# loop-Z/omniisaacgymenvs_loop

Hardware: AMD Instinct MI355X
Metric: env-steps/sec USV_CaptureXY at 1/2/4/8 MI355X; wall-clock to reward=30 (higher is better)
Workload: dtype fp32; 1 GPU; USV_Virtual_CaptureXY num_envs=131072/GPU PPO-MLP fp32 (BASELINE configs[4] per GPU: 2^20 envs over 8 GPUs); num_envs_per_gpu=131072, horizon_length=16, minibatch_size=8192, mini_epochs=8, parallelism=dp1, exchange=none (one rank), seed=0, full=False

## Files before the change

### omniisaacgymenvs_loop_amd/csrc/usv_field.hip

```cpp
#include "usv_device.h"

USV_PROBE_DEFINE(field)

namespace {

constexpr int G = USV_GRID;
constexpr int G2 = USV_GRID2;
constexpr int FS = USV_FIELD_STRIDE;
constexpr int T = 10;
constexpr int NT = G / T;
constexpr int kWaveThreads = 256;
constexpr int kMaxIters = 4096;
constexpr int kSlotStride = USV_FIELD_SLOT_STATS;
constexpr int kSlotObst = 160;
static_assert(kSlotObst + 2 * USV_NOBST <= kSlotStride, "slot_stats layout");
constexpr int kFieldPackMinEnvs = 32768;
#ifndef USV_SWEEP_WAVES
#define USV_SWEEP_WAVES 2
#endif
constexpr int kPackGrid = 256 * USV_SWEEP_WAVES;

enum {
  SS_GMIN_F = 0, SS_GMAX_F, SS_ANY_INF,
  SS_JMIN_F_NI, SS_JMAX_F_NI, SS_JMAX_F_ALL,
  SS_JRMIN_I_NI, SS_JRMAX_I_NI, SS_JRMAX_I_ALL,
  SS_INSIDE, SS_ITERS, SS_EXACT
};

__device__ __forceinline__ float wall(const uint32_t *freem, int bit) {
  const uint32_t f = (freem[bit >> 5] >> (bit & 31)) & 1u;
  return __uint_as_float((f - 1u) & 0x7f800000u);
}

constexpr int NTP = NT + 2;
constexpr uint32_t kInfBits = 0x7f800000u;
constexpr uint32_t kOcc = 0xFFFFFFFFu;
enum { E_TOP = 0, E_BOT, E_LEFT, E_RIGHT };
constexpr int kOccColWords = (G + 31) / 32;
__device__ __forceinline__ bool occ_bit(const uint32_t *occ, int r, int cc) {
  return (occ[cc * kOccColWords + (r >> 5)] >> (r & 31)) & 1u;
}

constexpr int kRefSweeps = (G * 3) / 2;
template <int NT>
__device__ __forceinline__ void cost_sweeps_exact(const uint32_t *occ, int ix, int iy, float *A, float *B) {
  const int tid = threadIdx.x;
  for (int q = tid; q < G2; q += NT) A[q] = (q == iy * G + ix) ? 0.f : INFINITY;
  __syncthreads();
  for (int it = 0; it < kRefSweeps; ++it) {
    for (int q = tid; q < G2; q += NT) {
      const int r = q / G, cc = q % G;
      float m = A[q];
#pragma unroll
      for (int dy = -1; dy <= 1; ++dy)
#pragma unroll
        for (int dx = -1; dx <= 1; ++dx) {
          if (!dx && !dy) continue;
          const int rr = r - dy, c2 = cc - dx;
          if (rr < 0 || rr >= G || c2 < 0 || c2 >= G) continue;
          m = fminf(m, A[rr * G + c2] + ((dx && dy) ? 1.414f : 1.0f));
        }
      const bool o = r == 0 || r == G - 1 || cc == 0 || cc == G - 1 || occ_bit(occ, r, cc);
      B[q] = o ? INFINITY : m;
    }
    __syncthreads();
    float *t = A; A = B; B = t;
  }
}

constexpr int kPlaceTB = 256;
__global__ __launch_bounds__(kPlaceTB) void k_field_place(usv_cfg_t c, usv_bufs_t b) {
  if (b.ctl[USV_CTL_PLACE] == 0) return;
  const int n = b.n;
  const int count = min(b.ctl[USV_CTL_RESET_COUNT], n);
  const uint64_t h_seed = (uint64_t)(uint32_t)b.ctl[USV_CTL_H_SEED_LO] | ((uint64_t)(uint32_t)b.ctl[USV_CTL_H_SEED_HI] << 32);
  const uint64_t h_step = (uint64_t)(uint32_t)b.ctl[USV_CTL_H_STEP_LO] | ((uint64_t)(uint32_t)b.ctl[USV_CTL_H_STEP_HI] << 32);
  const float *h_inj = reinterpret_cast<const float *>(
      (uintptr_t)((uint64_t)(uint32_t)b.ctl[USV_CTL_H_INJ_LO] | ((uint64_t)(uint32_t)b.ctl[USV_CTL_H_INJ_HI] << 32)));
  const int lane = threadIdx.x & 63;
  const int waves = (int)gridDim.x * (kPlaceTB / 64);
  for (int slot = (int)blockIdx.x * (kPlaceTB / 64) + (int)(threadIdx.x >> 6); slot < count; slot += waves) {
    const int e = b.reset_ids[slot];
    const float2 oc = place_obstacles(c, e, b.px[e], b.py[e], b.field_old_tgt[e], b.field_old_tgt[n + e], h_seed,
                                      h_step, h_inj);
    if (lane < USV_NOBST) {
      b.obst[(size_t)(2 * lane) * n + e] = oc.x;
      b.obst[(size_t)(2 * lane + 1) * n + e] = oc.y;
    }
  }
}

#define USV_SWEEP_NOTE(hb, m) (chg = __builtin_amdgcn_bitop3_b32(chg, (uint32_t)(hb), (uint32_t)(m), 0xF6))
template <bool kPlace, int TH = T, int TW = T, int NTHR = kWaveThreads>
__device__ __forceinline__ void field_wave_body(const usv_cfg_t &c, const usv_bufs_t &b) {
  constexpr int NTR = G / TH, NTC = G / TW;
  constexpr int NPR = NTR + 2, NPC = NTC + 2;
  constexpr int WC = NTHR / 128;
  static_assert(G % TH == 0 && G % TW == 0 && NTR <= 16 && NTC <= 8 * WC && NTHR % 128 == 0, "sweep tiling");
  static_assert(USV_FIELD_TH == TH && USV_FIELD_TW % TW == 0, "sweep tiles inside the field tiles");
  __shared__ uint32_t occ[G * kOccColWords];
  __shared__ float edgeh[2][NPR * NPC][TW];
  __shared__ float edgev[2][NPR * NPC][TH];
  __shared__ int lastc[NPR * NPC];
  __shared__ float so[2 * USV_NOBST];
  __shared__ float slin[G];
  const int n = b.n;
  const int count = min(b.ctl[USV_CTL_RESET_COUNT], n);
  const int tid = threadIdx.x;
  const int lane = tid & 63, wid = tid >> 6;
  const bool place = kPlace && b.ctl[USV_CTL_PLACE] != 0;
  uint64_t h_seed = 0, h_step = 0;
  const float *h_inj = nullptr;
  if (kPlace) {
    h_seed = (uint64_t)(uint32_t)b.ctl[USV_CTL_H_SEED_LO] | ((uint64_t)(uint32_t)b.ctl[USV_CTL_H_SEED_HI] << 32);
    h_step = (uint64_t)(uint32_t)b.ctl[USV_CTL_H_STEP_LO] | ((uint64_t)(uint32_t)b.ctl[USV_CTL_H_STEP_HI] << 32);
    h_inj = reinterpret_cast<const float *>(
        (uintptr_t)((uint64_t)(uint32_t)b.ctl[USV_CTL_H_INJ_LO] | ((uint64_t)(uint32_t)b.ctl[USV_CTL_H_INJ_HI] << 32)));
  }
  const int quad = tid >> 6, qk = tid & 63;
  const int qr = quad / WC, qc = quad % WC;
  const int qw = min(8, NTC - 8 * qc), qh = min(8, NTR - 8 * qr);
  const bool tile_ok = qk < qw * qh;
  const int tr = tile_ok ? qr * 8 + qk / qw : 0;
  const int tc = tile_ok ? qc * 8 + qk % qw : 0;
  const int r0 = tr * TH, c0 = tc * TW;
  const int tp = (tr + 1) * NPC + tc + 1;
  const float cell = (float)((double)c.map_size / G);
  const float half_map = (float)((double)c.map_size / 2);
  const float inv_r = (float)(1.0 / (double)c.influence_radius);
  for (int q = tid; q < 2 * NPR * NPC * TW; q += NTHR) {
    const int t = (q / TW) % (NPR * NPC);
    const int rr = t / NPC, cc = t % NPC;
    if (rr == 0 || rr == NPR - 1 || cc == 0 || cc == NPC - 1) (&edgeh[0][0][0])[q] = INFINITY;
  }
  for (int q = tid; q < 2 * NPR * NPC * TH; q += NTHR) {
    const int t = (q / TH) % (NPR * NPC);
    const int rr = t / NPC, cc = t % NPC;
    if (rr == 0 || rr == NPR - 1 || cc == 0 || cc == NPC - 1) (&edgev[0][0][0])[q] = INFINITY;
  }
  for (int q = tid; q < NPR * NPC; q += NTHR) lastc[q] = -1000;
  for (int slot = blockIdx.x; slot < count; slot += gridDim.x) {
    USV_PHASE(field, 0);
    const int e = b.reset_ids[slot];
    if (kPlace && place) {
      if (wid == 0) {
        const float2 oc = place_obstacles(c, e, b.px[e], b.py[e], b.field_old_tgt[e], b.field_old_tgt[n + e],
                                          h_seed, h_step, h_inj);
        if (lane < USV_NOBST) {
          so[2 * lane] = oc.x;
          so[2 * lane + 1] = oc.y;
          b.obst[(size_t)(2 * lane) * n + e] = oc.x;
          b.obst[(size_t)(2 * lane + 1) * n + e] = oc.y;
        }
      }
    } else if (tid < 2 * USV_NOBST) {
      so[tid] = b.obst[(size_t)tid * n + e];
    }
    if (tid < G) slin[tid] = grid_coord(b.grid_lin, c.map_size, tid);
    for (int q = tid; q < G * kOccColWords; q += NTHR) occ[q] = 0u;
    __syncthreads();
#ifdef USV_PHASE_PROBE
    if (tid == 0 && blockIdx.x < 4096) g_probe_field[blockIdx.x][12] = wall_clock64();
#endif
    if (tid < 2 * USV_NOBST) b.slot_stats[(size_t)slot * kSlotStride + kSlotObst + tid] = so[tid];
    {
      const float half_m = (float)((double)c.map_size / 2);
      const float cellf = (float)((double)c.map_size / G);
      const int reach = (int)ceilf(c.obstacle_radius / cellf) + 2;
      const int bw = 2 * reach + 1;
      for (int q = tid; q < USV_NOBST * bw * bw; q += NTHR) {
        const int o = q / (bw * bw), k = q % (bw * bw);
        const float ox = so[2 * o], oy = so[2 * o + 1];
        const float ic = (ox + half_m) / cellf - 0.5f, jc = (oy + half_m) / cellf - 0.5f;
        if (!(fabsf(ic) < 4.0f * G && fabsf(jc) < 4.0f * G)) continue;
        const int cc = (int)floorf(ic) - reach + k % bw, r = (int)floorf(jc) - reach + k / bw;
        if (cc < 0 || cc >= G || r < 0 || r >= G) continue;
        const float dx = slin[cc] - ox, dy = slin[r] - oy;
        if (sqrtf(fmaf(dy, dy, dx * dx)) - c.obstacle_radius <= 0.f)
          atomicOr(&occ[cc * kOccColWords + (r >> 5)], 1u << (r & 31));
      }
    }
    __syncthreads();
    USV_PHASE(field, 1);
#ifdef USV_PHASE_PROBE
    if (tid == 0 && blockIdx.x < 4096) g_probe_field[blockIdx.x][13] = clock64();
#endif
    const float tx = b.field_old_tgt[e], ty = b.field_old_tgt[n + e];
    int ix = (int)((tx + half_map) / cell), iy = (int)((ty + half_map) / cell);
    ix = min(max(ix, 0), G - 1);
    iy = min(max(iy, 0), G - 1);
    const bool tgt_free = !occ_bit(occ, iy, ix) && ix > 0 && ix < G - 1 && iy > 0 && iy < G - 1;
    float h[TH + 2][TW + 2];
    if (tile_ok) {
#pragma unroll
      for (int i = 0; i < TH; ++i)
#pragma unroll
        for (int j = 0; j < TW; ++j) {
          const int r = r0 + i, cc = c0 + j;
          const bool border = r == 0 || r == G - 1 || cc == 0 || cc == G - 1;
          const bool o = border || occ_bit(occ, r, cc);
          float init = INFINITY;
          if (o) {
            init = __uint_as_float(kOcc);
          } else if (tgt_free) {
            if (r == iy && cc == ix) init = 0.f;
          } else {
            const int di = r - iy, dj = cc - ix;
            if (abs(di) <= 1 && abs(dj) <= 1 && (di || dj)) init = (di && dj) ? 1.414f : 1.0f;
          }
          h[i + 1][j + 1] = init;
        }
#pragma unroll
      for (int k = 0; k < TW; ++k) {
        edgeh[E_TOP][tp][k] = h[1][k + 1];
        edgeh[E_BOT][tp][k] = h[TH][k + 1];
      }
#pragma unroll
      for (int k = 0; k < TH; ++k) {
        edgev[E_LEFT - 2][tp][k] = h[k + 1][1];
        edgev[E_RIGHT - 2][tp][k] = h[k + 1][TW];
      }
      lastc[tp] = 0;
    }
    __syncthreads();
    int it = 0;
    for (; it < kMaxIters; ++it) {
      int changed = 0;
      uint32_t chg = 0u;
      bool dirty = false;
      if (tile_ok) {
#pragma unroll
        for (int dr = -1; dr <= 1; ++dr)
#pragma unroll
          for (int dc = -1; dc <= 1; ++dc) dirty |= lastc[tp + dr * NPC + dc] >= it - 1;
      }
      if (dirty) {
#pragma unroll
        for (int k = 0; k < TW; ++k) {
          h[0][k + 1] = edgeh[E_BOT][tp - NPC][k];
          h[TH + 1][k + 1] = edgeh[E_TOP][tp + NPC][k];
        }
#pragma unroll
        for (int k = 0; k < TH; ++k) {
          h[k + 1][0] = edgev[E_RIGHT - 2][tp - 1][k];
          h[k + 1][TW + 1] = edgev[E_LEFT - 2][tp + 1][k];
        }
        h[0][0] = edgeh[E_BOT][tp - NPC - 1][TW - 1];
        h[0][TW + 1] = edgeh[E_BOT][tp - NPC + 1][0];
        h[TH + 1][0] = edgeh[E_TOP][tp + NPC - 1][TW - 1];
        h[TH + 1][TW + 1] = edgeh[E_TOP][tp + NPC + 1][0];
#pragma unroll
        for (int L = 0; L < 2 * TH + TW - 2; ++L)
#pragma unroll
          for (int i = 1; i <= TH; ++i) {
            const int j = L - 2 * (i - 1) + 1;
            if (j < 1 || j > TW) continue;
            const int32_t hb = __float_as_int(h[i][j]);
            int32_t m = min(hb, __float_as_int(fabsf(h[i - 1][j - 1]) + 1.414f));
            m = min(m, __float_as_int(fabsf(h[i - 1][j]) + 1.0f));
            m = min(m, __float_as_int(fabsf(h[i - 1][j + 1]) + 1.414f));
            m = min(m, __float_as_int(fabsf(h[i][j - 1]) + 1.0f));
            if (i == 1 || i == TH || j == 1 || j == TW) USV_SWEEP_NOTE(hb, m);
            h[i][j] = __int_as_float(m);
          }
#pragma unroll
        for (int L = 0; L < 2 * TH + TW - 2; ++L)
#pragma unroll
          for (int i = TH; i >= 1; --i) {
            const int j = TW - (L - 2 * (TH - i));
            if (j < 1 || j > TW) continue;
            const int32_t hb = __float_as_int(h[i][j]);
            int32_t m = min(hb, __float_as_int(fabsf(h[i + 1][j + 1]) + 1.414f));
            m = min(m, __float_as_int(fabsf(h[i + 1][j]) + 1.0f));
            m = min(m, __float_as_int(fabsf(h[i + 1][j - 1]) + 1.414f));
            m = min(m, __float_as_int(fabsf(h[i][j + 1]) + 1.0f));
            USV_SWEEP_NOTE(hb, m);
            h[i][j] = __int_as_float(m);
          }
        __asm__("" : "+v"(chg));
        changed = chg != 0u;
        if (changed) {
#pragma unroll
          for (int k = 0; k < TW; ++k) {
            edgeh[E_TOP][tp][k] = h[1][k + 1];
            edgeh[E_BOT][tp][k] = h[TH][k + 1];
          }
#pragma unroll
          for (int k = 0; k < TH; ++k) {
            edgev[E_LEFT - 2][tp][k] = h[k + 1][1];
            edgev[E_RIGHT - 2][tp][k] = h[k + 1][TW];
          }
          lastc[tp] = it;
        }
      }
      if (!__syncthreads_or(changed)) break;
    }
    USV_PHASE(field, 2);
#ifdef USV_PHASE_PROBE
    if (tid == 0 && blockIdx.x < 4096) g_probe_field[blockIdx.x][14] = clock64();
#endif
    constexpr float kPinnedCost = 224.0f;
    float hmax = 0.f;
    if (tile_ok) {
#pragma unroll
      for (int i = 0; i < TH; ++i)
#pragma unroll
        for (int j = 0; j < TW; ++j) {
          const uint32_t hb = __float_as_uint(h[i + 1][j + 1]);
          if (hb < kInfBits) hmax = fmaxf(hmax, h[i + 1][j + 1]);
        }
    }
    const bool exact = __syncthreads_or((hmax > kPinnedCost) || (it >= kMaxIters)) != 0;
    constexpr int kSub = USV_FIELD_TW / TW;
    static_assert(USV_FIELD_TCOLS * USV_FIELD_TW == G && USV_FIELD_TCOLS == NTC / kSub, "field tiles = sweep tiles");
    if (tile_ok) {
      float *Ft = b.field + (size_t)e * FS + (tr * USV_FIELD_TCOLS + tc / kSub) * (USV_FIELD_TH * USV_FIELD_TW) +
                  (tc % kSub) * TW;
#pragma unroll
      for (int i = 0; i < TH; ++i)
#pragma unroll
        for (int j = 0; j < TW; ++j)
          Ft[i * USV_FIELD_TW + j] = __float_as_uint(h[i + 1][j + 1]) > kInfBits ? INFINITY : h[i + 1][j + 1];
    }
    if (tile_ok) lastc[tp] = -1000;
    if (exact) {
      __syncthreads();
      float *Fe = b.field + (size_t)e * FS;
      float *scratch = b.sdf + (size_t)e * FS;
      cost_sweeps_exact<NTHR>(occ, ix, iy, Fe, scratch);
      for (int q = tid; q < G2; q += NTHR) Fe[field_idx(q / G, q % G)] = scratch[q];
      if (tid == 0) atomicAdd(&b.ctl[USV_CTL_FIELD_EXACT], 1);
    }
    if (tid == 0) {
      b.slot_stats[(size_t)slot * kSlotStride + SS_ITERS] = (float)it;
      b.slot_stats[(size_t)slot * kSlotStride + SS_EXACT] = exact ? 1.f : 0.f;
#ifdef USV_PHASE_PROBE
      if (blockIdx.x < 4096) g_probe_field[blockIdx.x][15] = (unsigned long long)it;
#endif
    }
    __syncthreads();
    USV_PHASE(field, 3);
  }
}

__global__ __launch_bounds__(kWaveThreads) void k_field_wave(usv_cfg_t c, usv_bufs_t b) { field_wave_body<true>(c, b); }
__global__ __launch_bounds__(kWaveThreads, USV_SWEEP_WAVES) void k_field_wave_pack(usv_cfg_t c, usv_bufs_t b) {
  field_wave_body<false>(c, b);
}
constexpr int kHalfThreads = 512;
__global__ __launch_bounds__(kHalfThreads) void k_field_wave_half(usv_cfg_t c, usv_bufs_t b) {
  field_wave_body<false, T, T / 2, kHalfThreads>(c, b);
}

struct BatchK {
  float inf_val, mask_inf;
};
__device__ __forceinline__ BatchK batch_k(const usv_cfg_t &c, const usv_bufs_t &b) {
  const float max_val = b.ctl[USV_CTL_ANY_FINITE] ? b.fscratch[0] : 100.0f;
  const float inf_val = max_val * 1.5f;
  const float cell = (float)((double)c.map_size / G);
  return BatchK{inf_val, goal_mask(c, inf_val, cell)};
}

#ifndef USV_STATS_WAVES
#define USV_STATS_WAVES 5
#endif
constexpr int kBandRows = 30, kBands = G / kBandRows;
constexpr int kRowGroups = 3;
constexpr int kWavePairs = 19;
constexpr int kBandIters = kBandRows / kRowGroups;
static_assert(G % kBandRows == 0 && kBandRows % kRowGroups == 0 && kWavePairs * kRowGroups <= 64 &&
              4 * 2 * kWavePairs >= G && G % 2 == 0, "k_field_stats geometry");
static_assert(kSlotObst >= 16 + 12 * kBands, "slot_stats band partials");
__global__ __launch_bounds__(256, USV_STATS_WAVES) void k_field_stats(usv_cfg_t c, usv_bufs_t b) {
  __shared__ float red[10][4];
  __shared__ int flags[2];
  __shared__ float slin[G];
  __shared__ float so[2 * USV_NOBST];
  const int count = min(b.ctl[USV_CTL_RESET_COUNT], b.n);
  const int tid = threadIdx.x, lane = tid & 63, wid = tid >> 6;
  const int cbase = wid * 2 * kWavePairs;
  const int cpl = lane % kWavePairs, rg = lane / kWavePairs;
  const int c0u = cbase + 2 * cpl;
  const bool act = rg < kRowGroups && c0u < G;
  const int c0 = act ? c0u : 0;
  const int rgc = act ? rg : 0;
  const int chi = min(cbase + 2 * kWavePairs - 1, G - 1);
  const float cell = (float)((double)c.map_size / G);
  const float inv_r = (float)(1.0 / (double)c.influence_radius);
  const float inv_safe = 1.0f / c.safe_radius;
  const float far_d = c.influence_radius + 2.0f * c.obstacle_radius + 0.01f * cell + 1e-3f;
  const uint32_t far2 = __float_as_uint(far_d * far_d);
  const int items = count * kBands;
  if (tid < G) slin[tid] = grid_coord(b.grid_lin, c.map_size, tid);
  const auto load_costs = [&](int wq, int eq, float2 *dst) {
    const float *F = b.field + (size_t)eq * FS;
#pragma unroll
    for (int k = 0; k < kBandIters; ++k) {
      const int r = (wq % kBands) * kBandRows + rgc + kRowGroups * k;
      dst[k] = *reinterpret_cast<const float2 *>(F + field_idx(r, c0));
    }
  };
  float2 gA[kBandIters];
  const auto item = [&](const int w, float2 (&gv)[kBandIters]) {
    const int slot = w / kBands, band = w % kBands;
    if (tid < 2 * USV_NOBST) so[tid] = b.slot_stats[(size_t)slot * kSlotStride + kSlotObst + tid];
    if (tid < 2) flags[tid] = 0;
    __syncthreads();
    load_costs(w, b.reset_ids[slot], gv);
    const float gxa = slin[c0], gxb = slin[c0 + 1];
    uint32_t omask;
    {
      const float ylo = slin[band * kBandRows], yhi = slin[band * kBandRows + kBandRows - 1];
      const float xlo = slin[cbase], xhi = slin[chi];
      const int ol = lane & (USV_NOBST - 1);
      const float oxl = so[2 * ol], oyl = so[2 * ol + 1];
      const float dyb = fmaxf(fmaxf(ylo - oyl, oyl - yhi), 0.f);
      const float dxb_ = fmaxf(fmaxf(xlo - oxl, oxl - xhi), 0.f);
      omask = (uint32_t)(__ballot(lane < USV_NOBST && !(dyb > far_d) && !(dxb_ > far_d)) & 0xFFFFull);
      omask = __builtin_amdgcn_readfirstlane(omask);
    }
    float gmin = INFINITY, gmax = -INFINITY, jmin_f = INFINITY, jmax_f = -INFINITY, jall_f = 0.f;
    float jrmin_i = INFINITY, jrmax_i = -INFINITY, jrall_i = 0.f;
    int any_inf = 0, inside = 0;
    const auto stat = [&](float g, float sv) {
      const float dte = sv - c.obstacle_radius;
      const bool ins = dte <= 0.f;
      inside |= ins;
      const float jr = j_raw(c, dte, inv_r);
      const bool gi = isinf(g);
      any_inf |= gi;
      const float j = jr * clampt(div_rn(g * cell, c.safe_radius, inv_safe), 0.f, 1.f);
      jrall_i = fmaxf(jrall_i, gi ? jr : 0.f);
      jrmin_i = fminf(jrmin_i, (gi && !ins) ? jr : INFINITY);
      jrmax_i = fmaxf(jrmax_i, (gi && !ins) ? jr : -INFINITY);
      gmin = fminf(gmin, gi ? INFINITY : g);
      gmax = fmaxf(gmax, gi ? -INFINITY : g);
      jall_f = fmaxf(jall_f, gi ? 0.f : j);
      jmin_f = fminf(jmin_f, (!gi && !ins) ? j : INFINITY);
      jmax_f = fmaxf(jmax_f, (!gi && !ins) ? j : -INFINITY);
    };
    const auto stat_far = [&](float g) {
      const bool gi = isinf(g);
      any_inf |= gi;
      jrmin_i = fminf(jrmin_i, gi ? 0.f : INFINITY);
      jrmax_i = fmaxf(jrmax_i, gi ? 0.f : -INFINITY);
      gmin = fminf(gmin, gi ? INFINITY : g);
      gmax = fmaxf(gmax, gi ? -INFINITY : g);
      jmin_f = fminf(jmin_f, gi ? INFINITY : 0.f);
      jmax_f = fmaxf(jmax_f, gi ? -INFINITY : 0.f);
    };
    float gy[kBandIters];
    uint32_t a[kBandIters], bb[kBandIters];
#pragma unroll
    for (int k = 0; k < kBandIters; ++k) {
      gy[k] = slin[band * kBandRows + rgc + kRowGroups * k];
      a[k] = bb[k] = 0x7F800000u;
    }
    for (uint32_t om = omask; om != 0u; om &= om - 1u) {
      const int o = __builtin_ctz(om);
      const float ox = so[2 * o], oyo = so[2 * o + 1];
      const float da = gxa - ox, db = gxb - ox;
      const float dxa = da * da, dxb = db * db;
#pragma unroll
      for (int k = 0; k < kBandIters; ++k) {
        const float dy = gy[k] - oyo;
        a[k] = min(a[k], __float_as_uint(fmaf(dy, dy, dxa)));
        bb[k] = min(bb[k], __float_as_uint(fmaf(dy, dy, dxb)));
      }
    }
#pragma unroll
    for (int k = 0; k < kBandIters; ++k) {
      const bool near = act && (a[k] < far2 || bb[k] < far2);
      if (__ballot(near) != 0ull) {
        const float sva = sqrtf(__uint_as_float(a[k])) - c.obstacle_radius;
        const float svb = sqrtf(__uint_as_float(bb[k])) - c.obstacle_radius;
        if (act) {
          stat(gv[k].x, sva);
          stat(gv[k].y, svb);
        }
      } else if (act) {
        stat_far(gv[k].x);
        stat_far(gv[k].y);
      }
    }
    float vals[9] = {wave_min(gmin), wave_max(gmax), wave_min(jmin_f), wave_max(jmax_f), wave_max(jall_f),
                     wave_min(jrmin_i), wave_max(jrmax_i), wave_max(jrall_i), 0.f};
    __syncthreads();
    if (lane == 0)
      for (int k = 0; k < 8; ++k) red[k][wid] = vals[k];
    if (any_inf) flags[0] = 1;
    if (inside) flags[1] = 1;
    __syncthreads();
    if (tid == 0) {
      float a[8];
      for (int k = 0; k < 8; ++k) a[k] = red[k][0];
      for (int v = 1; v < 4; ++v) {
        a[0] = fminf(a[0], red[0][v]); a[1] = fmaxf(a[1], red[1][v]);
        a[2] = fminf(a[2], red[2][v]); a[3] = fmaxf(a[3], red[3][v]); a[4] = fmaxf(a[4], red[4][v]);
        a[5] = fminf(a[5], red[5][v]); a[6] = fmaxf(a[6], red[6][v]); a[7] = fmaxf(a[7], red[7][v]);
      }
      float *pp = b.slot_stats + (size_t)slot * kSlotStride + 16 + 12 * band;
      pp[SS_GMIN_F] = a[0]; pp[SS_GMAX_F] = a[1]; pp[SS_ANY_INF] = flags[0] ? 1.f : 0.f;
      pp[SS_JMIN_F_NI] = a[2]; pp[SS_JMAX_F_NI] = a[3]; pp[SS_JMAX_F_ALL] = a[4];
      pp[SS_JRMIN_I_NI] = a[5]; pp[SS_JRMAX_I_NI] = a[6]; pp[SS_JRMAX_I_ALL] = a[7];
      pp[SS_INSIDE] = flags[1] ? 1.f : 0.f;
    }
    __syncthreads();
  };
  for (int w = blockIdx.x; w < items; w += gridDim.x) item(w, gA);
}

#ifndef USV_BATCH_BLOCKS
#define USV_BATCH_BLOCKS 64
#endif
#ifndef USV_BATCH_SLOTS_PER_WAVE
#define USV_BATCH_SLOTS_PER_WAVE 6
#endif
constexpr int kBatchBlocks = USV_BATCH_BLOCKS;
constexpr int kBatchSpw = USV_BATCH_SLOTS_PER_WAVE;
static_assert(kBatchSpw >= 1 && 10 * kBatchSpw <= 64, "k_field_batch lane groups");
__global__ __launch_bounds__(256) void k_field_batch(usv_cfg_t c, usv_bufs_t b) {
  __shared__ float wred[4][4];
  __shared__ bool last;
  const int count = min(b.ctl[USV_CTL_RESET_COUNT], b.n);
  if (count <= 0) return;
  const int tid = threadIdx.x, lane = tid & 63, wid = tid >> 6;
  const int grp = lane / 10, q = lane % 10, l0 = 10 * grp;
  const int nw = (int)gridDim.x * 4;
  float gfin = -INFINITY, jf = 0.f, jr = 0.f, ins = 0.f;
  const bool is_min = q == SS_GMIN_F || q == SS_JMIN_F_NI || q == SS_JRMIN_I_NI;
  for (int sl0 = ((int)blockIdx.x * 4 + wid) * kBatchSpw; sl0 < count; sl0 += nw * kBatchSpw) {
    const int sl = sl0 + grp;
    const bool ok = grp < kBatchSpw && sl < count;
    float a = 0.f;
    if (ok) {
      float *st = b.slot_stats + (size_t)sl * kSlotStride;
      float x[kBands];
#pragma unroll
      for (int ch = 0; ch < kBands; ++ch) x[ch] = st[16 + 12 * ch + q];
      a = x[0];
#pragma unroll
      for (int ch = 1; ch < kBands; ++ch) a = is_min ? fminf(a, x[ch]) : fmaxf(a, x[ch]);
      st[q] = a;
    }
    const float s_gmax = __shfl(a, ok ? l0 + SS_GMAX_F : lane, 64);
    const float s_anyinf = __shfl(a, ok ? l0 + SS_ANY_INF : lane, 64);
    const float s_jf = __shfl(a, ok ? l0 + SS_JMAX_F_ALL : lane, 64);
    const float s_jr = __shfl(a, ok ? l0 + SS_JRMAX_I_ALL : lane, 64);
    const float s_in = __shfl(a, ok ? l0 + SS_INSIDE : lane, 64);
    if (ok) {
      gfin = fmaxf(gfin, s_gmax);
      jf = fmaxf(jf, s_jf);
      if (s_anyinf != 0.f) jr = fmaxf(jr, s_jr);
      ins = fmaxf(ins, s_in);
    }
  }
  gfin = wave_max(gfin); jf = wave_max(jf); jr = wave_max(jr); ins = wave_max(ins);
  if (lane == 0) { wred[wid][0] = gfin; wred[wid][1] = jf; wred[wid][2] = jr; wred[wid][3] = ins; }
  __syncthreads();
  if (tid == 0) {
    float g = wred[0][0], f = wred[0][1], r = wred[0][2], in = wred[0][3];
    for (int w = 1; w < 4; ++w) {
      g = fmaxf(g, wred[w][0]); f = fmaxf(f, wred[w][1]); r = fmaxf(r, wred[w][2]); in = fmaxf(in, wred[w][3]);
    }
    if (isfinite(g)) {
      atomic_max_f32(&b.fscratch[0], g);
      atomicOr(&b.ctl[USV_CTL_ANY_FINITE], 1);
    }
    atomic_max_f32(&b.fscratch[2], f);
    atomic_max_f32(&b.fscratch[3], r);
    if (in != 0.f) atomicOr(&b.ctl[USV_CTL_ANY_INSIDE], 1);
    __threadfence();
    last = atomicAdd(&b.ctl[USV_CTL_BATCH_DONE], 1) == (int)gridDim.x - 1;
  }
  __syncthreads();
  if (!last || tid != 0) return;
  __threadfence();
  const BatchK k = batch_k(c, b);
  b.fscratch[1] = fmaxf(b.fscratch[2], b.fscratch[3] * k.mask_inf);
  b.ctl[USV_CTL_BATCH_DONE] = 0;
}

__global__ __launch_bounds__(256) void k_field_norm(usv_cfg_t c, usv_bufs_t b) {
  const int count = min(b.ctl[USV_CTL_RESET_COUNT], b.n);
  const BatchK k = batch_k(c, b);
  const bool any_inside = b.ctl[USV_CTL_ANY_INSIDE] != 0;
  const float cur_max = b.fscratch[1];
  const float high = (cur_max > 1e-6f) ? cur_max * 10.0f : 100.0f;
  for (int slot = (int)(blockIdx.x * blockDim.x + threadIdx.x); slot < count; slot += (int)(gridDim.x * blockDim.x)) {
    const int e = b.reset_ids[slot];
    const float *st = b.slot_stats + (size_t)slot * kSlotStride;
    const bool has_inf = st[SS_ANY_INF] != 0.f;
    const bool has_inside = st[SS_INSIDE] != 0.f;
    const float gmin = has_inf ? fminf(st[SS_GMIN_F], k.inf_val) : st[SS_GMIN_F];
    const float gmax = has_inf ? fmaxf(st[SS_GMAX_F], k.inf_val) : st[SS_GMAX_F];
    float jmn = st[SS_JMIN_F_NI], jmx = st[SS_JMAX_F_NI];
    if (isfinite(st[SS_JRMIN_I_NI])) {
      jmn = fminf(jmn, st[SS_JRMIN_I_NI] * k.mask_inf);
      jmx = fmaxf(jmx, st[SS_JRMAX_I_NI] * k.mask_inf);
    }
    if (any_inside && has_inside) { jmn = fminf(jmn, high); jmx = fmaxf(jmx, high); }
    float4 *fn = reinterpret_cast<float4 *>(b.fnorm + (size_t)e * USV_FNORM);
    const float gden = (gmax - gmin) + 1e-6f, jden = (jmx - jmn) + 1e-6f;
    fn[0] = make_float4(gmin, gden, jmn, jden);
    fn[1] = make_float4(k.inf_val, any_inside ? high : -high, 1.0f / gden, 1.0f / jden);
  }
}

__global__ __launch_bounds__(256) void k_field_view(usv_cfg_t c, usv_bufs_t b, const int32_t *ids, int count,
                                                    float *out) {
  const float cell = (float)((double)c.map_size / G);
  const float inv_r = (float)(1.0 / (double)c.influence_radius);
  const float inv_safe = 1.0f / c.safe_radius;
  const long long total = (long long)count * G2;
  for (long long q = (long long)blockIdx.x * blockDim.x + threadIdx.x; q < total; q += (long long)gridDim.x * blockDim.x) {
    const int i = (int)(q / G2), cell_i = (int)(q % G2), r = cell_i / G, cc = cell_i % G;
    const int e = ids[i];
    const float4 *fn = reinterpret_cast<const float4 *>(b.fnorm + (size_t)e * USV_FNORM);
    const FieldNorm k = field_norm_of(fn[0], fn[1]);
    const float *ob = b.obst + e;
    const float sv = cell_sdf([&](int o) { return make_float2(ob[(size_t)(2 * o) * b.n], ob[(size_t)(2 * o + 1) * b.n]); },
                              grid_coord(b.grid_lin, c.map_size, cc), grid_coord(b.grid_lin, c.map_size, r),
                              c.obstacle_radius);
    out[q] = field_value(c, k, sv, b.field[(size_t)e * FS + field_idx(r, cc)], cell, inv_r, inv_safe);
  }
}

}

namespace {
constexpr int kStatsGridCap = 4096;
static int stats_grid(int n) { return n * kBands < kStatsGridCap ? n * kBands : kStatsGridCap; }

int field_stages(const usv_cfg_t *cfg, const usv_bufs_t *b, int stage, hipStream_t s) {
  const int grid_b = b->n < 512 ? b->n : 512;
  const int grid_n = (b->n + 255) / 256 < 64 ? (b->n + 255) / 256 : 64;
  const int grid_p = (b->n + kPlaceTB / 64 - 1) / (kPlaceTB / 64) < 1024 ? (b->n + kPlaceTB / 64 - 1) / (kPlaceTB / 64) : 1024;
  if (stage == 1) {
    hipLaunchKernelGGL(k_field_place, dim3(grid_p), dim3(kPlaceTB), 0, s, *cfg, *b);
    USV_CHECK_LAUNCH();
    return 0;
  }
  if (stage == 2 || stage == 3) {
    const char *half_env = getenv("USV_FIELD_HALF");
    const bool half = half_env ? atoi(half_env) != 0 : b->n < kFieldPackMinEnvs;
    if (half) {
      hipLaunchKernelGGL(k_field_wave_half, dim3(b->n < 256 ? b->n : 256), dim3(kHalfThreads), 0, s, *cfg, *b);
    } else {
      const int grid_w = b->n < kPackGrid ? b->n : kPackGrid;
      hipLaunchKernelGGL(k_field_wave_pack, dim3(grid_w), dim3(kWaveThreads), 0, s, *cfg, *b);
    }
    USV_CHECK_LAUNCH();
    const int grid_s = stats_grid(b->n);
    hipLaunchKernelGGL(k_field_stats, dim3(grid_s), dim3(256), 0, s, *cfg, *b);
    USV_CHECK_LAUNCH();
  }
  if (stage == 2 || stage == 4) {
    hipLaunchKernelGGL(k_field_batch, dim3(kBatchBlocks), dim3(256), 0, s, *cfg, *b);
    USV_CHECK_LAUNCH();
    hipLaunchKernelGGL(k_field_norm, dim3(grid_n), dim3(256), 0, s, *cfg, *b);
    USV_CHECK_LAUNCH();
  }
  return 0;
}
}

extern "C" int usv_field_stage(const usv_cfg_t *cfg, const usv_bufs_t *b, int stage, void *stream) {
  if (!cfg || !b || b->n <= 0 || !b->slot_stats || !b->field || !b->sdf || !b->fnorm || stage < 1 || stage > 4) return 1;
  return field_stages(cfg, b, stage, (hipStream_t)stream);
}

extern "C" int usv_field_view(const usv_cfg_t *cfg, const usv_bufs_t *b, const int32_t *env_ids, int count,
                              float *out, void *stream) {
  if (!cfg || !b || b->n <= 0 || !b->field || !b->sdf || !b->fnorm || !env_ids || !out || count < 0) return 1;
  if (count == 0) return 0;
  const long long total = (long long)count * G2;
  const int grid = (int)((total + 255) / 256 < 8192 ? (total + 255) / 256 : 8192);
  hipLaunchKernelGGL(k_field_view, dim3(grid), dim3(256), 0, (hipStream_t)stream, *cfg, *b, env_ids, count, out);
  USV_CHECK_LAUNCH();
  return 0;
}

extern "C" int usv_potential_field(const usv_cfg_t *cfg, const usv_bufs_t *b, void *stream) {
  if (!cfg || !b || b->n <= 0 || !b->slot_stats || !b->field || !b->sdf || !b->fnorm) return 1;
  hipStream_t s = (hipStream_t)stream;
  const int grid_b = b->n < 512 ? b->n : 512;
  const int grid_n = (b->n + 255) / 256 < 64 ? (b->n + 255) / 256 : 64;
  const char *pack_env = getenv("USV_FIELD_PACK");
  const bool pack = pack_env ? atoi(pack_env) != 0 : b->n >= kFieldPackMinEnvs;
  if (pack) {
    const int grid_p = (b->n + kPlaceTB / 64 - 1) / (kPlaceTB / 64) < 1024 ? (b->n + kPlaceTB / 64 - 1) / (kPlaceTB / 64) : 1024;
    hipLaunchKernelGGL(k_field_place, dim3(grid_p), dim3(kPlaceTB), 0, s, *cfg, *b);
    USV_CHECK_LAUNCH();
  }
  if (pack) hipLaunchKernelGGL(k_field_wave_pack, dim3(b->n < kPackGrid ? b->n : kPackGrid), dim3(kWaveThreads), 0, s,
                              *cfg, *b);
  else hipLaunchKernelGGL(k_field_wave, dim3(grid_b), dim3(kWaveThreads), 0, s, *cfg, *b);
  USV_CHECK_LAUNCH();
  const int grid_s = stats_grid(b->n);
  hipLaunchKernelGGL(k_field_stats, dim3(grid_s), dim3(256), 0, s, *cfg, *b);
  USV_CHECK_LAUNCH();
  hipLaunchKernelGGL(k_field_batch, dim3(kBatchBlocks), dim3(256), 0, s, *cfg, *b);
  USV_CHECK_LAUNCH();
  hipLaunchKernelGGL(k_field_norm, dim3(grid_n), dim3(256), 0, s, *cfg, *b);
  USV_CHECK_LAUNCH();
  return 0;
}
```

Before: 37.11 million env-steps/s.

## Fold cost stats into wave kernel and restrict stats pass to obstacle windows

The wave solver now builds a near-obstacle bitmask and folds the cost-only statistics (min/max cost, inf flags) into its epilogue while the values are still in registers. The separate full-grid band stats kernel is replaced by a near-window kernel that only visits cells within the influence distance of each obstacle. Per-slot partials drop from many bands to two parts. This removes a full re-read of every reset env's field, at the cost of extra shared memory and reductions in the wave kernel, and the near kernel may revisit cells where obstacle windows overlap.

Result: faster. 37.52 million env-steps/s (median of 6 runs) (+1.1%).

```diff
diff --git a/omniisaacgymenvs_loop_amd/csrc/usv_field.hip b/omniisaacgymenvs_loop_amd/csrc/usv_field.hip
--- a/omniisaacgymenvs_loop_amd/csrc/usv_field.hip
+++ b/omniisaacgymenvs_loop_amd/csrc/usv_field.hip
@@ -13,7 +13,10 @@
 constexpr int kMaxIters = 4096;
 constexpr int kSlotStride = USV_FIELD_SLOT_STATS;
 constexpr int kSlotObst = 160;
-static_assert(kSlotObst + 2 * USV_NOBST <= kSlotStride, "slot_stats layout");
+constexpr int kSlotCost = 16, kSlotNear = 28;
+constexpr int kParts = 2;
+static_assert(kSlotObst + 2 * USV_NOBST <= kSlotStride && kSlotNear == kSlotCost + 12 &&
+              kSlotCost + 12 * kParts <= kSlotObst, "slot_stats layout");
 constexpr int kFieldPackMinEnvs = 32768;
 #ifndef USV_SWEEP_WAVES
 #define USV_SWEEP_WAVES 2
@@ -40,6 +43,39 @@
 __device__ __forceinline__ bool occ_bit(const uint32_t *occ, int r, int cc) {
   return (occ[cc * kOccColWords + (r >> 5)] >> (r & 31)) & 1u;
 }
+
+__device__ __forceinline__ float field_far_d(const usv_cfg_t &c, float cell) {
+  return c.influence_radius + 2.0f * c.obstacle_radius + 0.01f * cell + 1e-3f;
+}
+struct Win {
+  int cl, ch, rl, rh;
+};
+__device__ __forceinline__ Win near_window(float ox, float oy, float half_m, float cellf, float far_d) {
+  const float wc = (far_d + cellf) / cellf;
+  const float ic = (ox + half_m) / cellf - 0.5f, jc = (oy + half_m) / cellf - 0.5f;
+  Win w{1, 0, 1, 0};
+  if (!(fabsf(ic) < 4.0f * G && fabsf(jc) < 4.0f * G)) return w;
+  const int cl = max((int)ceilf(ic - wc), 0), ch = min((int)floorf(ic + wc), G - 1);
+  const int rl = max((int)ceilf(jc - wc), 0), rh = min((int)floorf(jc + wc), G - 1);
+  if (cl <= ch && rl <= rh) w = Win{cl, ch, rl, rh};
+  return w;
+}
+template <int kRows>
+__device__ __forceinline__ uint32_t col_bits(const uint32_t *map, int r0, int cc) {
+  static_assert(kRows <= 32, "one word of rows");
+  const int w = r0 >> 5;
+  const uint64_t lo = map[cc * kOccColWords + w], hi = map[cc * kOccColWords + min(w + 1, kOccColWords - 1)];
+  return (uint32_t)(((hi << 32) | lo) >> (r0 & 31)) & ((1u << kRows) - 1u);
+}
+struct CostFold {
+  uint32_t gmin = 0xFFFFFFFFu, amax = 0u, fmin = 0xFFFFFFFFu, fmax = 0u;
+  __device__ __forceinline__ void cell(uint32_t hb, uint32_t nm) {
+    gmin = min(gmin, hb);
+    amax = max(amax, hb);
+    fmin = min(fmin, hb | nm);
+    fmax = max(fmax, hb & ~nm);
+  }
+};
 
 constexpr int kRefSweeps = (G * 3) / 2;
 template <int NT>
@@ -99,6 +135,8 @@
   static_assert(G % TH == 0 && G % TW == 0 && NTR <= 16 && NTC <= 8 * WC && NTHR % 128 == 0, "sweep tiling");
   static_assert(USV_FIELD_TH == TH && USV_FIELD_TW % TW == 0, "sweep tiles inside the field tiles");
   __shared__ uint32_t occ[G * kOccColWords];
+  __shared__ uint32_t nearm[G * kOccColWords];
+  __shared__ float cred[5][NTHR / 64];
   __shared__ float edgeh[2][NPR * NPC][TW];
   __shared__ float edgev[2][NPR * NPC][TH];
   __shared__ int lastc[NPR * NPC];
@@ -157,7 +195,7 @@
       so[tid] = b.obst[(size_t)tid * n + e];
     }
     if (tid < G) slin[tid] = grid_coord(b.grid_lin, c.map_size, tid);
-    for (int q = tid; q < G * kOccColWords; q += NTHR) occ[q] = 0u;
+    for (int q = tid; q < G * kOccColWords; q += NTHR) occ[q] = nearm[q] = 0u;
     __syncthreads();
 #ifdef USV_PHASE_PROBE
     if (tid == 0 && blockIdx.x < 4096) g_probe_field[blockIdx.x][12] = wall_clock64();
@@ -179,6 +217,15 @@
         if (sqrtf(fmaf(dy, dy, dx * dx)) - c.obstacle_radius <= 0.f)
           atomicOr(&occ[cc * kOccColWords + (r >> 5)], 1u << (r & 31));
       }
+      static_assert((USV_NOBST & (USV_NOBST - 1)) == 0 && NTHR % USV_NOBST == 0, "near map threads");
+      const int o = tid & (USV_NOBST - 1);
+      const Win w = near_window(so[2 * o], so[2 * o + 1], half_m, cellf, field_far_d(c, cellf));
+      for (int cc = w.cl + tid / USV_NOBST; cc <= w.ch; cc += NTHR / USV_NOBST) {
+        for (int wi = w.rl >> 5; wi <= w.rh >> 5; ++wi) {
+          const int lo = max(w.rl, 32 * wi), hi = min(w.rh, 32 * wi + 31);
+          atomicOr(&nearm[cc * kOccColWords + wi], (uint32_t)(((1ull << (hi - lo + 1)) - 1ull) << (lo & 31)));
+        }
+      }
     }
     __syncthreads();
     USV_PHASE(field, 1);
@@ -301,14 +348,18 @@
 #endif
     constexpr float kPinnedCost = 224.0f;
     float hmax = 0.f;
+    CostFold cf;
     if (tile_ok) {
 #pragma unroll
-      for (int i = 0; i < TH; ++i)
-#pragma unroll
-        for (int j = 0; j < TW; ++j) {
+      for (int j = 0; j < TW; ++j) {
+        const uint32_t nb = col_bits<TH>(nearm, r0, c0 + j);
+#pragma unroll
+        for (int i = 0; i < TH; ++i) {
           const uint32_t hb = __float_as_uint(h[i + 1][j + 1]);
           if (hb < kInfBits) hmax = fmaxf(hmax, h[i + 1][j + 1]);
-        }
+          cf.cell(hb, (uint32_t)__builtin_amdgcn_sbfe(nb, i, 1));
+        }
+      }
     }
     const bool exact = __syncthreads_or((hmax > kPinnedCost) || (it >= kMaxIters)) != 0;
     constexpr int kSub = USV_FIELD_TW / TW;
@@ -328,17 +379,47 @@
       float *Fe = b.field + (size_t)e * FS;
       float *scratch = b.sdf + (size_t)e * FS;
       cost_sweeps_exact<NTHR>(occ, ix, iy, Fe, scratch);
-      for (int q = tid; q < G2; q += NTHR) Fe[field_idx(q / G, q % G)] = scratch[q];
+      cf = CostFold{};
+      hmax = 0.f;
+      for (int q = tid; q < G2; q += NTHR) {
+        const float v = scratch[q];
+        const int r = q / G, cc = q % G;
+        Fe[field_idx(r, cc)] = v;
+        if (__float_as_uint(v) < kInfBits) hmax = fmaxf(hmax, v);
+        cf.cell(__float_as_uint(v), occ_bit(nearm, r, cc) ? 0xFFFFFFFFu : 0u);
+      }
       if (tid == 0) atomicAdd(&b.ctl[USV_CTL_FIELD_EXACT], 1);
     }
+    {
+      const bool fin = cf.gmin < kInfBits;
+      const float v0 = wave_min(fin ? __uint_as_float(cf.gmin) : INFINITY);
+      const float v1 = wave_max(fin ? hmax : -INFINITY);
+      const float v2 = wave_max(cf.amax >= kInfBits ? 1.f : 0.f);
+      const float v3 = wave_min(cf.fmin < kInfBits ? 0.f : INFINITY);
+      const float v4 = wave_min(cf.fmax >= kInfBits ? 0.f : INFINITY);
+      if (lane == 0) {
+        cred[0][wid] = v0; cred[1][wid] = v1; cred[2][wid] = v2; cred[3][wid] = v3; cred[4][wid] = v4;
+      }
+    }
+    __syncthreads();
     if (tid == 0) {
+      float a[5];
+      for (int k = 0; k < 5; ++k) a[k] = cred[k][0];
+      for (int v = 1; v < NTHR / 64; ++v) {
+        a[0] = fminf(a[0], cred[0][v]); a[1] = fmaxf(a[1], cred[1][v]); a[2] = fmaxf(a[2], cred[2][v]);
+        a[3] = fminf(a[3], cred[3][v]); a[4] = fminf(a[4], cred[4][v]);
+      }
+      float *pp = b.slot_stats + (size_t)slot * kSlotStride + kSlotCost;
+      pp[SS_GMIN_F] = a[0]; pp[SS_GMAX_F] = a[1]; pp[SS_ANY_INF] = a[2];
+      pp[SS_JMIN_F_NI] = a[3]; pp[SS_JMAX_F_NI] = a[3] == 0.f ? 0.f : -INFINITY; pp[SS_JMAX_F_ALL] = 0.f;
+      pp[SS_JRMIN_I_NI] = a[4]; pp[SS_JRMAX_I_NI] = a[4] == 0.f ? 0.f : -INFINITY; pp[SS_JRMAX_I_ALL] = 0.f;
+      pp[SS_INSIDE] = 0.f;
       b.slot_stats[(size_t)slot * kSlotStride + SS_ITERS] = (float)it;
       b.slot_stats[(size_t)slot * kSlotStride + SS_EXACT] = exact ? 1.f : 0.f;
 #ifdef USV_PHASE_PROBE
       if (blockIdx.x < 4096) g_probe_field[blockIdx.x][15] = (unsigned long long)it;
 #endif
     }
-    __syncthreads();
     USV_PHASE(field, 3);
   }
 }
@@ -362,153 +443,125 @@
   return BatchK{inf_val, goal_mask(c, inf_val, cell)};
 }
 
-#ifndef USV_STATS_WAVES
-#define USV_STATS_WAVES 5
-#endif
-constexpr int kBandRows = 30, kBands = G / kBandRows;
-constexpr int kRowGroups = 3;
-constexpr int kWavePairs = 19;
-constexpr int kBandIters = kBandRows / kRowGroups;
-static_assert(G % kBandRows == 0 && kBandRows % kRowGroups == 0 && kWavePairs * kRowGroups <= 64 &&
-              4 * 2 * kWavePairs >= G && G % 2 == 0, "k_field_stats geometry");
-static_assert(kSlotObst >= 16 + 12 * kBands, "slot_stats band partials");
-__global__ __launch_bounds__(256, USV_STATS_WAVES) void k_field_stats(usv_cfg_t c, usv_bufs_t b) {
-  __shared__ float red[10][4];
-  __shared__ int flags[2];
+constexpr int kNearWaves = 4;
+constexpr int kNearCells = 8;
+__global__ __launch_bounds__(64 * kNearWaves) void k_field_near(usv_cfg_t c, usv_bufs_t b) {
+  __shared__ float red[6][kNearWaves];
+  __shared__ int flag[kNearWaves];
   __shared__ float slin[G];
   __shared__ float so[2 * USV_NOBST];
   const int count = min(b.ctl[USV_CTL_RESET_COUNT], b.n);
   const int tid = threadIdx.x, lane = tid & 63, wid = tid >> 6;
-  const int cbase = wid * 2 * kWavePairs;
-  const int cpl = lane % kWavePairs, rg = lane / kWavePairs;
-  const int c0u = cbase + 2 * cpl;
-  const bool act = rg < kRowGroups && c0u < G;
-  const int c0 = act ? c0u : 0;
-  const int rgc = act ? rg : 0;
-  const int chi = min(cbase + 2 * kWavePairs - 1, G - 1);
   const float cell = (float)((double)c.map_size / G);
+  const float half_m = (float)((double)c.map_size / 2);
   const float inv_r = (float)(1.0 / (double)c.influence_radius);
   const float inv_safe = 1.0f / c.safe_radius;
-  const float far_d = c.influence_radius + 2.0f * c.obstacle_radius + 0.01f * cell + 1e-3f;
+  const float far_d = field_far_d(c, cell);
   const uint32_t far2 = __float_as_uint(far_d * far_d);
-  const int items = count * kBands;
   if (tid < G) slin[tid] = grid_coord(b.grid_lin, c.map_size, tid);
-  const auto load_costs = [&](int wq, int eq, float2 *dst) {
-    const float *F = b.field + (size_t)eq * FS;
-#pragma unroll
-    for (int k = 0; k < kBandIters; ++k) {
-      const int r = (wq % kBands) * kBandRows + rgc + kRowGroups * k;
-      dst[k] = *reinterpret_cast<const float2 *>(F + field_idx(r, c0));
-    }
-  };
-  float2 gA[kBandIters];
-  const auto item = [&](const int w, float2 (&gv)[kBandIters]) {
-    const int slot = w / kBands, band = w % kBands;
+  for (int slot = blockIdx.x; slot < count; slot += gridDim.x) {
     if (tid < 2 * USV_NOBST) so[tid] = b.slot_stats[(size_t)slot * kSlotStride + kSlotObst + tid];
-    if (tid < 2) flags[tid] = 0;
+    const float *F = b.field + (size_t)b.reset_ids[slot] * FS;
     __syncthreads();
-    load_costs(w, b.reset_ids[slot], gv);
-    const float gxa = slin[c0], gxb = slin[c0 + 1];
-    uint32_t omask;
-    {
-      const float ylo = slin[band * kBandRows], yhi = slin[band * kBandRows + kBandRows - 1];
-      const float xlo = slin[cbase], xhi = slin[chi];
-      const int ol = lane & (USV_NOBST - 1);
-      const float oxl = so[2 * ol], oyl = so[2 * ol + 1];
-      const float dyb = fmaxf(fmaxf(ylo - oyl, oyl - yhi), 0.f);
-      const float dxb_ = fmaxf(fmaxf(xlo - oxl, oxl - xhi), 0.f);
-      omask = (uint32_t)(__ballot(lane < USV_NOBST && !(dyb > far_d) && !(dxb_ > far_d)) & 0xFFFFull);
-      omask = __builtin_amdgcn_readfirstlane(omask);
-    }
-    float gmin = INFINITY, gmax = -INFINITY, jmin_f = INFINITY, jmax_f = -INFINITY, jall_f = 0.f;
+    float jmin_f = INFINITY, jmax_f = -INFINITY, jall_f = 0.f;
     float jrmin_i = INFINITY, jrmax_i = -INFINITY, jrall_i = 0.f;
-    int any_inf = 0, inside = 0;
+    int inside = 0;
     const auto stat = [&](float g, float sv) {
       const float dte = sv - c.obstacle_radius;
       const bool ins = dte <= 0.f;
       inside |= ins;
       const float jr = j_raw(c, dte, inv_r);
       const bool gi = isinf(g);
-      any_inf |= gi;
       const float j = jr * clampt(div_rn(g * cell, c.safe_radius, inv_safe), 0.f, 1.f);
       jrall_i = fmaxf(jrall_i, gi ? jr : 0.f);
       jrmin_i = fminf(jrmin_i, (gi && !ins) ? jr : INFINITY);
       jrmax_i = fmaxf(jrmax_i, (gi && !ins) ? jr : -INFINITY);
-      gmin = fminf(gmin, gi ? INFINITY : g);
-      gmax = fmaxf(gmax, gi ? -INFINITY : g);
       jall_f = fmaxf(jall_f, gi ? 0.f : j);
       jmin_f = fminf(jmin_f, (!gi && !ins) ? j : INFINITY);
       jmax_f = fmaxf(jmax_f, (!gi && !ins) ? j : -INFINITY);
     };
     const auto stat_far = [&](float g) {
       const bool gi = isinf(g);
-      any_inf |= gi;
       jrmin_i = fminf(jrmin_i, gi ? 0.f : INFINITY);
       jrmax_i = fmaxf(jrmax_i, gi ? 0.f : -INFINITY);
-      gmin = fminf(gmin, gi ? INFINITY : g);
-      gmax = fmaxf(gmax, gi ? -INFINITY : g);
       jmin_f = fminf(jmin_f, gi ? INFINITY : 0.f);
       jmax_f = fmaxf(jmax_f, gi ? -INFINITY : 0.f);
     };
-    float gy[kBandIters];
-    uint32_t a[kBandIters], bb[kBandIters];
-#pragma unroll
-    for (int k = 0; k < kBandIters; ++k) {
-      gy[k] = slin[band * kBandRows + rgc + kRowGroups * k];
-      a[k] = bb[k] = 0x7F800000u;
-    }
-    for (uint32_t om = omask; om != 0u; om &= om - 1u) {
-      const int o = __builtin_ctz(om);
-      const float ox = so[2 * o], oyo = so[2 * o + 1];
-      const float da = gxa - ox, db = gxb - ox;
-      const float dxa = da * da, dxb = db * db;
-#pragma unroll
-      for (int k = 0; k < kBandIters; ++k) {
-        const float dy = gy[k] - oyo;
-        a[k] = min(a[k], __float_as_uint(fmaf(dy, dy, dxa)));
-        bb[k] = min(bb[k], __float_as_uint(fmaf(dy, dy, dxb)));
-      }
-    }
-#pragma unroll
-    for (int k = 0; k < kBandIters; ++k) {
-      const bool near = act && (a[k] < far2 || bb[k] < far2);
-      if (__ballot(near) != 0ull) {
-        const float sva = sqrtf(__uint_as_float(a[k])) - c.obstacle_radius;
-        const float svb = sqrtf(__uint_as_float(bb[k])) - c.obstacle_radius;
-        if (act) {
-          stat(gv[k].x, sva);
-          stat(gv[k].y, svb);
-        }
-      } else if (act) {
-        stat_far(gv[k].x);
-        stat_far(gv[k].y);
-      }
-    }
-    float vals[9] = {wave_min(gmin), wave_max(gmax), wave_min(jmin_f), wave_max(jmax_f), wave_max(jall_f),
-                     wave_min(jrmin_i), wave_max(jrmax_i), wave_max(jrall_i), 0.f};
-    __syncthreads();
-    if (lane == 0)
-      for (int k = 0; k < 8; ++k) red[k][wid] = vals[k];
-    if (any_inf) flags[0] = 1;
-    if (inside) flags[1] = 1;
+    for (int o = wid; o < USV_NOBST; o += kNearWaves) {
+      const Win w = near_window(so[2 * o], so[2 * o + 1], half_m, cell, far_d);
+      if (w.cl > w.ch) continue;
+      const int ww = w.ch - w.cl + 1, area = ww * (w.rh - w.rl + 1);
+      const float inv_ww = 1.0f / (float)ww;
+      uint32_t omask;
+      {
+        const float ylo = slin[w.rl], yhi = slin[w.rh], xlo = slin[w.cl], xhi = slin[w.ch];
+        const int ol = lane & (USV_NOBST - 1);
+        const float oxl = so[2 * ol], oyl = so[2 * ol + 1];
+        const float dyb = fmaxf(fmaxf(ylo - oyl, oyl - yhi), 0.f);
+        const float dxb = fmaxf(fmaxf(xlo - oxl, oxl - xhi), 0.f);
+        omask = (uint32_t)(__ballot(lane < USV_NOBST && !(dyb > far_d) && !(dxb > far_d)) & 0xFFFFull);
+        omask = __builtin_amdgcn_readfirstlane(omask);
+      }
+      for (int k0 = 0; k0 < area; k0 += 64 * kNearCells) {
+        float g[kNearCells], gx[kNearCells], gy[kNearCells];
+        uint32_t a[kNearCells];
+        bool ok[kNearCells];
+#pragma unroll
+        for (int u = 0; u < kNearCells; ++u) {
+          const int k = k0 + 64 * u + lane;
+          ok[u] = k < area;
+          const int kr = ok[u] ? (int)(((float)k + 0.5f) * inv_ww) : 0;
+          const int r = w.rl + kr, cc = w.cl + (ok[u] ? k - kr * ww : 0);
+          g[u] = F[field_idx(r, cc)];
+          gx[u] = slin[cc];
+          gy[u] = slin[r];
+          a[u] = 0x7F800000u;
+        }
+        for (uint32_t om = omask; om != 0u; om &= om - 1u) {
+          const int p = __builtin_ctz(om);
+          const float ox = so[2 * p], oy = so[2 * p + 1];
+#pragma unroll
+          for (int u = 0; u < kNearCells; ++u) {
+            const float dx = gx[u] - ox, dy = gy[u] - oy;
+            a[u] = min(a[u], __float_as_uint(fmaf(dy, dy, dx * dx)));
+          }
+        }
+#pragma unroll
+        for (int u = 0; u < kNearCells; ++u) {
+          const bool near = ok[u] && a[u] < far2;
+          if (__ballot(near) != 0ull) {
+            const float sv = sqrtf(__uint_as_float(a[u])) - c.obstacle_radius;
+            if (ok[u]) stat(g[u], sv);
+          } else if (ok[u]) {
+            stat_far(g[u]);
+          }
+        }
+      }
+    }
+    const float v0 = wave_min(jmin_f), v1 = wave_max(jmax_f), v2 = wave_max(jall_f);
+    const float v3 = wave_min(jrmin_i), v4 = wave_max(jrmax_i), v5 = wave_max(jrall_i);
+    const bool ins_w = __ballot(inside != 0) != 0ull;
+    if (lane == 0) {
+      red[0][wid] = v0; red[1][wid] = v1; red[2][wid] = v2; red[3][wid] = v3; red[4][wid] = v4; red[5][wid] = v5;
+      flag[wid] = ins_w;
+    }
     __syncthreads();
     if (tid == 0) {
-      float a[8];
-      for (int k = 0; k < 8; ++k) a[k] = red[k][0];
-      for (int v = 1; v < 4; ++v) {
-        a[0] = fminf(a[0], red[0][v]); a[1] = fmaxf(a[1], red[1][v]);
-        a[2] = fminf(a[2], red[2][v]); a[3] = fmaxf(a[3], red[3][v]); a[4] = fmaxf(a[4], red[4][v]);
-        a[5] = fminf(a[5], red[5][v]); a[6] = fmaxf(a[6], red[6][v]); a[7] = fmaxf(a[7], red[7][v]);
-      }
-      float *pp = b.slot_stats + (size_t)slot * kSlotStride + 16 + 12 * band;
-      pp[SS_GMIN_F] = a[0]; pp[SS_GMAX_F] = a[1]; pp[SS_ANY_INF] = flags[0] ? 1.f : 0.f;
-      pp[SS_JMIN_F_NI] = a[2]; pp[SS_JMAX_F_NI] = a[3]; pp[SS_JMAX_F_ALL] = a[4];
-      pp[SS_JRMIN_I_NI] = a[5]; pp[SS_JRMAX_I_NI] = a[6]; pp[SS_JRMAX_I_ALL] = a[7];
-      pp[SS_INSIDE] = flags[1] ? 1.f : 0.f;
-    }
-    __syncthreads();
-  };
-  for (int w = blockIdx.x; w < items; w += gridDim.x) item(w, gA);
+      float r[6];
+      int in = flag[0];
+      for (int k = 0; k < 6; ++k) r[k] = red[k][0];
+      for (int v = 1; v < kNearWaves; ++v) {
+        r[0] = fminf(r[0], red[0][v]); r[1] = fmaxf(r[1], red[1][v]); r[2] = fmaxf(r[2], red[2][v]);
+        r[3] = fminf(r[3], red[3][v]); r[4] = fmaxf(r[4], red[4][v]); r[5] = fmaxf(r[5], red[5][v]);
+        in |= flag[v];
+      }
+      float *pp = b.slot_stats + (size_t)slot * kSlotStride + kSlotNear;
+      pp[SS_GMIN_F] = INFINITY; pp[SS_GMAX_F] = -INFINITY; pp[SS_ANY_INF] = 0.f;
+      pp[SS_JMIN_F_NI] = r[0]; pp[SS_JMAX_F_NI] = r[1]; pp[SS_JMAX_F_ALL] = r[2];
+      pp[SS_JRMIN_I_NI] = r[3]; pp[SS_JRMAX_I_NI] = r[4]; pp[SS_JRMAX_I_ALL] = r[5];
+      pp[SS_INSIDE] = in ? 1.f : 0.f;
+    }
+  }
 }
 
 #ifndef USV_BATCH_BLOCKS
@@ -536,12 +589,12 @@
     float a = 0.f;
     if (ok) {
       float *st = b.slot_stats + (size_t)sl * kSlotStride;
-      float x[kBands];
-#pragma unroll
-      for (int ch = 0; ch < kBands; ++ch) x[ch] = st[16 + 12 * ch + q];
+      float x[kParts];
+#pragma unroll
+      for (int ch = 0; ch < kParts; ++ch) x[ch] = st[kSlotCost + 12 * ch + q];
       a = x[0];
 #pragma unroll
-      for (int ch = 1; ch < kBands; ++ch) a = is_min ? fminf(a, x[ch]) : fmaxf(a, x[ch]);
+      for (int ch = 1; ch < kParts; ++ch) a = is_min ? fminf(a, x[ch]) : fmaxf(a, x[ch]);
       st[q] = a;
     }
     const float s_gmax = __shfl(a, ok ? l0 + SS_GMAX_F : lane, 64);
@@ -630,8 +683,8 @@
 }
 
 namespace {
-constexpr int kStatsGridCap = 4096;
-static int stats_grid(int n) { return n * kBands < kStatsGridCap ? n * kBands : kStatsGridCap; }
+constexpr int kNearGridCap = 2048;
+static int near_grid(int n) { return n < kNearGridCap ? n : kNearGridCap; }
 
 int field_stages(const usv_cfg_t *cfg, const usv_bufs_t *b, int stage, hipStream_t s) {
   const int grid_b = b->n < 512 ? b->n : 512;
@@ -652,8 +705,7 @@
       hipLaunchKernelGGL(k_field_wave_pack, dim3(grid_w), dim3(kWaveThreads), 0, s, *cfg, *b);
     }
     USV_CHECK_LAUNCH();
-    const int grid_s = stats_grid(b->n);
-    hipLaunchKernelGGL(k_field_stats, dim3(grid_s), dim3(256), 0, s, *cfg, *b);
+    hipLaunchKernelGGL(k_field_near, dim3(near_grid(b->n)), dim3(64 * kNearWaves), 0, s, *cfg, *b);
     USV_CHECK_LAUNCH();
   }
   if (stage == 2 || stage == 4) {
@@ -698,8 +750,7 @@
                               *cfg, *b);
   else hipLaunchKernelGGL(k_field_wave, dim3(grid_b), dim3(kWaveThreads), 0, s, *cfg, *b);
   USV_CHECK_LAUNCH();
-  const int grid_s = stats_grid(b->n);
-  hipLaunchKernelGGL(k_field_stats, dim3(grid_s), dim3(256), 0, s, *cfg, *b);
+  hipLaunchKernelGGL(k_field_near, dim3(near_grid(b->n)), dim3(64 * kNearWaves), 0, s, *cfg, *b);
   USV_CHECK_LAUNCH();
   hipLaunchKernelGGL(k_field_batch, dim3(kBatchBlocks), dim3(256), 0, s, *cfg, *b);
   USV_CHECK_LAUNCH();
```
